# Maryamsana-1998/DiffCodec-Controlling-Latent-Diffusion-for-Perceptual-Video-Compression

Measured on AMD Instinct MI355X. Metric: decoded frames/sec @ 512x512, 20-step DDIM, GOP-12, higher is better.
Workload: dtype bf16; 1 GPU; 512x512 inter frames of a GOP-12 clip, 16 per step per GPU, 20-step DDIM, CFG 4.5 (model batch 32), control scale 1.7, SD-1.5 + DualFlowControlNet + VAE decode, random-init weights; hip_graphs=True, parallelism=unit-shard x1, backend=none, backend_world_size=1

## Files before the change

### diffcodec-controlling-latent-diffusion-for-perceptual-video-compression_amd/blocks.py

```python
import torch

from . import ops
from .ops import PackedConv


PROJ_IN_FUSE_MIN_ROWS = 1 << 62
PROJ_IN_GN_ON_LOAD = True
LN_FOLD = True


BUFFER_EPOCH = [0]


def _f32(sd, key, device):
    return sd[key].detach().float().contiguous().to(device)


class TimeEmbedding:

    def __init__(self, sd, device, ch0, resnet_prefixes):
        self.ch0 = ch0
        self.l1 = PackedConv(sd["time_embedding.linear_1.weight"], sd["time_embedding.linear_1.bias"], device)
        self.l2 = PackedConv(sd["time_embedding.linear_2.weight"], sd["time_embedding.linear_2.bias"], device)
        ws, bs, self.slices, off = [], [], {}, 0
# ... 19 lines not shown


class ResnetBlock:

    def __init__(self, sd, p, device, groups, eps):
        self.p, self.groups, self.eps = p, groups, eps
        self.n1 = (_f32(sd, p + "norm1.weight", device), _f32(sd, p + "norm1.bias", device))
        self.n2 = (_f32(sd, p + "norm2.weight", device), _f32(sd, p + "norm2.bias", device))
        self.conv1 = PackedConv(sd[p + "conv1.weight"], sd[p + "conv1.bias"], device)
        self.conv2 = PackedConv(sd[p + "conv2.weight"], sd[p + "conv2.bias"], device)
        self.shortcut = None
        if p + "conv_shortcut.weight" in sd:
            self.shortcut = PackedConv(sd[p + "conv_shortcut.weight"], sd[p + "conv_shortcut.bias"], device)

    def __call__(self, x, temb=None, x2=None):
        ab1 = ops.group_norm_ab(x, self.n1[0], self.n1[1], self.groups, self.eps, x2=x2)
        h = ops.conv_gn_silu(x, self.conv1, ab1, x2=x2, row_add=None if temb is None else temb.slice(self.p, x.shape[0]),
                             gn_part=True)
        ab2 = ops.group_norm_ab(h, self.n2[0], self.n2[1], self.groups, self.eps)
        if self.shortcut is not None:
            sc = ops.conv(x, self.shortcut, x2=x2)
        else:
            assert x2 is None
            sc = x
        return ops.conv_gn_silu(h, self.conv2, ab2, residual=sc, gn_part=True)


class TransformerBlock:

    def __init__(self, sd, p, device, heads, groups):
        self.heads, self.groups = heads, groups
        self.norm = (_f32(sd, p + "norm.weight", device), _f32(sd, p + "norm.bias", device))
        self.proj_in = PackedConv(sd[p + "proj_in.weight"], sd[p + "proj_in.bias"], device)
        self.proj_out = PackedConv(sd[p + "proj_out.weight"], sd[p + "proj_out.bias"], device)
        q = p + "transformer_blocks.0."
        self.ln = [(_f32(sd, q + f"norm{i}.weight", device), _f32(sd, q + f"norm{i}.bias", device)) for i in (1, 2, 3)]
        self.fold = LN_FOLD

        def ln(i):
            return (sd[q + f"norm{i}.weight"], sd[q + f"norm{i}.bias"], 1e-5) if self.fold else None
# ... 12 lines not shown
        new = ops.linear(ctx_bf16, self.kv2)
        if self.kv_ctx is not None and self.kv_ctx.shape == new.shape:
            self.kv_ctx.copy_(new)
        else:
            self.kv_ctx = new
            BUFFER_EPOCH[0] += 1

    def __call__(self, x, cfg_shared=False):
        n, h, w, c = x.shape
        fold = self.fold
        parts = ops.row_stats_parts(c) if fold else 0

        def stats_buf(rows):
            return torch.empty((rows, parts, 2), device=x.device, dtype=torch.float32) if fold else None

        ab = ops.group_norm_ab(x, self.norm[0], self.norm[1], self.groups, 1e-6)
        if PROJ_IN_GN_ON_LOAD and self.proj_in.bias is not None and ops.rowpanel_takes(n * h * w, h * w, c, self.proj_in.cout):
            st = stats_buf(n * h * w)
            t = ops.conv(x, self.proj_in, gn_ab=ab, gn_silu=False, stats_out=st).reshape(n, h * w, c)
        elif n * h * w > PROJ_IN_FUSE_MIN_ROWS:
            t = ops.conv(x, self.proj_in, gn_ab=ab, gn_silu=False).reshape(n, h * w, c)
            st = ops.row_stats(t) if fold else None
        else:
            st = stats_buf(n * h * w)
            t = ops.conv(ops.gn_apply(x, ab), self.proj_in, stats_out=st).reshape(n, h * w, c)
        qkv = ops.linear(t, self.qkv1, ln_partials=(st, 1e-5)) if fold else ops.linear(ops.layer_norm(t, *self.ln[0]), self.qkv1)
        a = ops.attention(qkv[..., :c], qkv[..., c:2 * c], qkv[..., 2 * c:], self.heads)
        st = stats_buf(n * h * w)
        t = ops.linear(a, self.out1, residual=t, stats_out=st)
        q = ops.linear(t, self.q2, ln_partials=(st, 1e-5)) if fold else ops.linear(ops.layer_norm(t, *self.ln[1]), self.q2)
        kv = self.kv_ctx
        if not cfg_shared:
            a = ops.attention(q, kv[..., :c], kv[..., c:], self.heads)
            st = stats_buf(n * h * w)
            t = ops.linear(a, self.out2, residual=t, stats_out=st)
        else:
            assert kv.shape[0] == 2 * n, "cfg_shared needs the [uncond | cond] context batch"
            a = torch.empty((2 * n, h * w, c), device=x.device, dtype=x.dtype)
            t2 = torch.empty_like(a)
            st = stats_buf(2 * n * h * w)
# ... 79 lines not shown
```

### diffcodec-controlling-latent-diffusion-for-perceptual-video-compression_amd/csrc/dc_conv_route.h

```cpp
#pragma once
#include "dc_common.h"
#include "../../include/diffcodec_hip.h"

struct dc_route {
    int kernel;
    int variant;
    int epi;
    int splitk;
    int ln_first;
    int tm, tn;
    int nst;
    int st;
    int gn;
    int ks3;
    int fast, ups, sh;
    int gn_chunks;
};

#define DC_ROUTE_PASS 1

static inline int dc_n_tile(const dc_conv_desc& d) { return (d.Cout % 160 == 0 && d.epilogue == 0) ? 160 : 128; }

int dc_gemm_dma_route(const dc_conv_desc& d, dc_route& r);
int dc_gemm_dma_launch(const dc_conv_desc& d, const dc_route& r, hipStream_t st);
int dc_gemm_rowpanel_route(const dc_conv_desc& d, dc_route& r);
int dc_gemm_rowpanel_launch(const dc_conv_desc& d, const dc_route& r, hipStream_t st);
int dc_gemm_p8_route(const dc_conv_desc& d, dc_route& r);
int dc_gemm_p8_launch(const dc_conv_desc& d, const dc_route& r, hipStream_t st);
int dc_gemm_wide_route(const dc_conv_desc& d, dc_route& r);
int dc_gemm_wide_launch(const dc_conv_desc& d, const dc_route& r, hipStream_t st);
int dc_conv3x3_tile_route(const dc_conv_desc& d, dc_route& r);
int dc_conv3x3_tile_launch(const dc_conv_desc& d, const dc_route& r, hipStream_t st);
```

### diffcodec-controlling-latent-diffusion-for-perceptual-video-compression_amd/csrc/igemm.hip

```cpp
#include "dc_conv_route.h"

namespace {

constexpr int BK = 64;

template <int WM, int WN, int TM, int TN, bool KS3, bool GN>
__global__ __launch_bounds__(256, 2) void igemm_kernel(const dc_conv_desc d)
{
    constexpr int BM = WM * TM * 16;
    constexpr int BN = WN * TN * 16;
    constexpr int PA = BM / 32;
    constexpr int PB = BN / 32;
    constexpr int A_BYTES = BM * 128;
    constexpr int B_BYTES = BN * 128;
    constexpr int BUF_BYTES = A_BYTES + B_BYTES;
    static_assert(WM * WN == 4, "4 waves");
    extern __shared__ __attribute__((aligned(16))) char smem[];

    const int tid = threadIdx.x;
    const int lane = tid & 63;
    const int wave = tid >> 6;
    const int wm = wave % WM;
    const int wn = wave / WM;
    const int q = tid & 7;
// ... 365 lines not shown
    if (d.row_add_stride == 0) d.row_add_stride = d.Cout;
    if (d.epilogue == 1 && (d.splitk > 1 || (d.Cout & 31) || d.residual || d.row_add || d.out_f32)) return DC_ERR_INVALID;
    const int asked = d.splitk, nkc = Cin >> 6;
    d.splitk = r.splitk = splitk_fixpoint(asked, nkc);
    int rc = dc_gemm_dma_route(d, r);
    if (rc == DC_ROUTE_PASS) rc = dc_conv3x3_tile_route(d, r);
    if (rc == DC_ROUTE_PASS) {
        d.splitk = r.splitk = splitk_fixpoint(asked, (d.ksize == 3 ? 9 : 1) * nkc);
        rc = igemm_route(d, r);
    }
    if (rc != DC_OK) return rc;
    if ((d.Cout & 15) && !(r.kernel == DC_ROUTE_CONV3X3_TILE && asked == 1)) return DC_ERR_INVALID;
    const bool gemm = r.kernel != DC_ROUTE_CONV3X3_TILE && r.kernel != DC_ROUTE_IGEMM;
    if ((d.ln_stats || d.stats_out) && !gemm) return DC_ERR_INVALID;
    if (d.gn_part_out && r.gn_chunks == 0) return DC_ERR_INVALID;
    return DC_OK;
}

}

extern "C" int dc_conv_gn_part_chunks(const dc_conv_desc* dp)
{
    if (!dp || dp->splitk > 1) return 0;
    dc_conv_desc q = *dp, d;
    if (!q.gn_part_out) q.gn_part_out = (float*)(uintptr_t)16;
    dc_route r;
    return conv_route(q, d, r) == DC_OK ? r.gn_chunks : 0;
}

extern "C" long long dc_conv_igemm_ws_bytes(const dc_conv_desc* d)
// ... 57 lines not shown
        rc = dc_ln_finalize(d.ln_stats, d.ln_scratch, (long long)d.N * d.Ho * d.Wo, d.ln_parts, d.C1 + d.C2, d.ln_eps, stream);
        if (rc != DC_OK) return rc;
        d.ln_stats = d.ln_scratch;
        d.ln_parts = 0;
    }
    switch (r.kernel) {
        case DC_ROUTE_GEMM_DMA: rc = dc_gemm_dma_launch(d, r, st); break;
        case DC_ROUTE_GEMM_WIDE: rc = dc_gemm_wide_launch(d, r, st); break;
        case DC_ROUTE_GEMM_P8: rc = dc_gemm_p8_launch(d, r, st); break;
        case DC_ROUTE_GEMM_ROWPANEL: rc = dc_gemm_rowpanel_launch(d, r, st); break;
        case DC_ROUTE_CONV3X3_TILE: rc = dc_conv3x3_tile_launch(d, r, st); break;
        default: rc = igemm_launch(d, r, st); break;
    }
    if (rc != DC_OK) return rc;
    if (d.splitk > 1) {
        const long long M = (long long)d.N * d.Ho * d.Wo;
        const long long total4 = M * d.Cout / 4;
        hipLaunchKernelGGL(splitk_finish_kernel, dim3(dc_cdiv(total4, 256)), dim3(256), 0, st, d, total4);
        return dc_launch_status();
    }
    return DC_OK;
}
```

### diffcodec-controlling-latent-diffusion-for-perceptual-video-compression_amd/csrc/norm.hip

```cpp
#include "dc_common.h"
#include "../../include/diffcodec_hip.h"

namespace {

__global__ __launch_bounds__(256) void gn_stats_kernel(const bf16_t* __restrict__ x, float* __restrict__ part,
                                                       long long HW, int C, int pix_per_block, int N)
{
    extern __shared__ float red[];
    const int nv = C >> 3;
    const int n = blockIdx.y;
    const long long p_begin = (long long)blockIdx.x * pix_per_block;
    const long long p_end = min(HW, p_begin + pix_per_block);
    const int tpp = min(nv, 256);
    const int ppb = 256 / tpp;
    const int vl = threadIdx.x % tpp, pl = threadIdx.x / tpp;
    if (pl < ppb) {
        for (int v = vl; v < nv; v += tpp) {
            float s[8], ss[8];
#pragma unroll
            for (int j = 0; j < 8; ++j) s[j] = ss[j] = 0.f;
            for (long long p0 = p_begin + pl; p0 < p_end; p0 += 4LL * ppb) {
                u32x4 raw[4];
#pragma unroll
                for (int u = 0; u < 4; ++u) {
// ... 175 lines not shown
                        continue;
                    }
                    float lo = __uint_as_float(raw[u][j] << 16) * g[j][0] + g[j][1];
                    float hi = __uint_as_float(raw[u][j] & 0xffff0000u) * g[j][2] + g[j][3];
                    lo = dc_silu(lo);
                    hi = dc_silu(hi);
                    bf16x2 pk = {(bf16_t)lo, (bf16_t)hi};
                    o[j] = *(uint32_t*)&pk;
                }
                *(u32x4*)(dst + p * C) = u32x4{o[0], o[1], o[2], o[3]};
            }
        }
    }
}

__global__ __launch_bounds__(256) void fdn_modulate_kernel(const bf16_t* __restrict__ x, const float* __restrict__ ab,
                                                           const bf16_t* __restrict__ gamma,
                                                           const bf16_t* __restrict__ beta, bf16_t* __restrict__ y,
                                                           int Bp, long long HW, int C, long long total_vec)
{
    const int nv = C >> 3;
    for (long long i = (long long)blockIdx.x * 256 + threadIdx.x; i < total_vec; i += (long long)gridDim.x * 256) {
        const long long pix = i / nv;
        const int c = (int)(i - pix * nv) * 8;
        const int n = (int)(pix / HW);
        const long long ppix = (long long)(n % Bp) * HW + (pix - (long long)n * HW);
        const bf16x8 xv = *(const bf16x8*)(x + pix * C + c);
        const bf16x8 gv = *(const bf16x8*)(gamma + ppix * C + c);
        const bf16x8 bv = *(const bf16x8*)(beta + ppix * C + c);
        const float* abp = ab + ((long long)n * C + c) * 2;
// ... 118 lines not shown
    if (!x1 || !ab || !y || N <= 0 || HW <= 0 || (C1 & 7) || (C2 & 7) || (C2 && !x2)) return DC_ERR_INVALID;
    const int nv = C >> 3, tpp = nv < 256 ? nv : 256, ppb = 256 / tpp;
    long long chunks = HW / (16LL * ppb);
    if (chunks < 1) chunks = 1;
    while (chunks * N < 1024 && chunks * 2 * 4 * ppb <= HW) chunks *= 2;
    const long long cap = 4096 / N > 0 ? 4096 / N : 1;
    if (chunks > cap) chunks = cap;
    if (chunks < 1) chunks = 1;
    const int pix_per_block = (int)((HW + chunks - 1) / chunks);
    const dim3 grid((unsigned)dc_cdiv(HW, pix_per_block), N);
    hipLaunchKernelGGL(gn_apply_kernel, grid, dim3(256), 0, (hipStream_t)stream, (const bf16_t*)x1, C1, (const bf16_t*)x2, C2, ab,
                       (bf16_t*)y, HW, pix_per_block, silu);
    return dc_launch_status();
}

extern "C" int dc_fdn_modulate_nhwc_bf16(const void* x, const float* ab, const void* gamma, const void* beta, void* y,
                                         int N, int Bp, long long HW, int C, void* stream)
{
    if (!x || !ab || !gamma || !beta || !y || N <= 0 || Bp <= 0 || HW <= 0 || (C & 7)) return DC_ERR_INVALID;
    const long long total_vec = (long long)N * HW * (C >> 3);
    const int grid = (int)min((long long)4096, (total_vec + 255) / 256);
    hipLaunchKernelGGL(fdn_modulate_kernel, dim3(grid), dim3(256), 0, (hipStream_t)stream, (const bf16_t*)x, ab,
                       (const bf16_t*)gamma, (const bf16_t*)beta, (bf16_t*)y, Bp, HW, C, total_vec);
    return dc_launch_status();
}

__global__ __launch_bounds__(256) void row_stats_kernel(const bf16_t* __restrict__ x, float* __restrict__ stats, long long M, int C)
{
    const int lane = threadIdx.x & 63;
    const long long row = (long long)blockIdx.x * 4 + (threadIdx.x >> 6);
// ... 57 lines not shown
```

### diffcodec-controlling-latent-diffusion-for-perceptual-video-compression_amd/lib.py

```python
import ctypes
import os
from ctypes import POINTER, c_double, c_float, c_int, c_longlong, c_void_p

HERE = os.path.dirname(os.path.abspath(__file__))
LIB_PATH = os.path.join(HERE, "libdiffcodec_hip.so")

vp, i32, i64, f32, f64 = c_void_p, c_int, c_longlong, c_float, c_double


class ConvDesc(ctypes.Structure):
    _fields_ = [
        ("x1", vp), ("x2", vp), ("w", vp), ("bias", vp), ("gn_ab", vp), ("row_add", vp), ("residual", vp),
        ("out", vp), ("splitk_ws", vp),
        ("N", i32), ("H", i32), ("W", i32), ("C1", i32), ("C2", i32), ("Cout", i32),
        ("ksize", i32), ("stride", i32), ("pad", i32), ("upsample", i32), ("Ho", i32), ("Wo", i32),
        ("gn_silu", i32), ("epilogue", i32), ("out_f32", i32), ("out_scale", f32), ("splitk", i32), ("gn_batch", i32),
        ("act", i32), ("row_add_stride", i64),
        ("ln_stats", vp), ("ln_colsum", vp), ("stats_out", vp), ("gn_part_out", vp),
        ("ln_parts", i32), ("ln_eps", f32), ("ln_scratch", vp),
    ]


SIGNATURES = {
    "dc_splat_soft_f32": [vp, vp, vp, vp, vp, vp, i32, i32, i32, i32, vp],
    "dc_splat_sum_f32": [vp, vp, vp, vp, i32, i32, i32, i32, vp],
    "dc_splat_ws_bytes": [i32, i32, i32],
    "dc_occlusion_mask_f32": [vp, vp, vp, vp, i32, i32, i32, vp],
    "dc_flow_resize_normalize_f32": [vp, i64, vp, i32, i32, i32, i32, i32, vp],
    "dc_flow_resize_divide_f32": [vp, i64, vp, i32, i32, i32, i32, i32, f32, f32, vp],
    "dc_fuse_warped_f32": [vp, vp, vp, vp, vp, vp, vp, i32, i32, i32, i32, vp],
    "dc_conv3x3_nchw_f32": [vp, i64, vp, vp, vp, i32, i32, i32, i32, i32, i32, i32, vp],
    "dc_conv3x3_f32_route": [i32, i32, i32, i32, i32, POINTER(i32)],
    "dc_nchw_f32_to_nhwc_bf16": [vp, vp, i32, i32, i32, i32, vp],
    "dc_nhwc_bf16_to_nchw_f32": [vp, vp, i32, i32, i32, i32, vp],
# ... 2 lines not shown
    "dc_conv_igemm_bf16": [POINTER(ConvDesc), vp],
    "dc_conv_route": [POINTER(ConvDesc), POINTER(i32)],
    "dc_conv_instance": [POINTER(ConvDesc), POINTER(i32)],
    "dc_conv_igemm_ws_bytes": [POINTER(ConvDesc)],
    "dc_gemm_row_stats_parts": [i32],
    "dc_conv_gn_part_chunks": [POINTER(ConvDesc)],
    "dc_row_stats_bf16": [vp, vp, i64, i32, vp],
    "dc_ln_finalize": [vp, vp, i64, i32, i32, f32, vp],
    "dc_conv_small_cin_bf16": [vp, vp, vp, vp, i32, i32, i32, i32, i32, i32, i32, i32, i32, i32, vp],
    "dc_conv_small_cout_bf16": [vp, vp, vp, vp, i32, i32, vp, i32, i32, i32, i32, i32, i32, i32, vp],
    "dc_gn_stats_nhwc_bf16": [vp, vp, i32, i64, i32, vp],
    "dc_gn_stats_chunks": [i64, i32],
    "dc_gn_finalize": [vp, i32, i32, vp, i32, i32, vp, vp, vp, i32, i32, i64, f32, vp],
    "dc_gn_direct_nhwc_bf16": [vp, i32, vp, i32, vp, vp, vp, i32, i64, i32, f32, vp],
    "dc_gn_apply_nhwc_bf16": [vp, i32, vp, i32, vp, vp, i32, i64, i32, vp],
    "dc_fdn_modulate_nhwc_bf16": [vp, vp, vp, vp, vp, i32, i32, i64, i32, vp],
    "dc_layernorm_bf16": [vp, vp, vp, vp, i64, i32, f32, vp],
    "dc_attention_bf16": [vp, vp, vp, vp, i32, i32, i32, i32, i32, i64, i64, i64, i64, f32, vp],
    "dc_attention_route": [i32, i32, i32, i32, i32, POINTER(i32)],
    "dc_attention_causal_small_bf16": [vp, vp, vp, vp, i32, i32, i32, i32, i64, i64, i64, i64, f32, vp],
    "dc_embed_tokens_bf16": [vp, vp, vp, vp, i32, i32, i32, i32, vp],
    "dc_softmax_rows_f32_to_bf16": [vp, vp, i64, i32, f32, vp],
    "dc_timestep_embedding_f32": [vp, vp, vp, i32, i32, vp],
    "dc_freeu_lowfreq_nhwc_bf16": [vp, vp, i32, i32, i32, i32, f32, vp],
    "dc_freeu_backbone_nhwc_bf16": [vp, vp, i64, i32, f32, vp],
    "dc_lincomb4_f32": [vp, vp, vp, vp, f32, f32, f32, f32, vp, i64, vp],
    "dc_transpose_bf16": [vp, vp, i32, i32, i32, vp],
    "dc_vae_sample_latents": [vp, vp, vp, f32, i32, i32, i32, i32, vp],
    "dc_silu_f32": [vp, vp, i64, vp],
    "dc_add_bf16": [vp, vp, vp, i64, vp],
# ... 105 lines not shown
```

### diffcodec-controlling-latent-diffusion-for-perceptual-video-compression_amd/ops.py

```python
import collections
import ctypes
import math

import torch

from . import lib
from .lib import ConvDesc

BF16 = torch.bfloat16
F32 = torch.float32


def _meta(family, shape, flops, nbytes):
    return (family, shape, float(flops), float(nbytes)) if lib.TIMER is not None else None



GN_DIRECT_MAX_PIXELS = 256
GN_EPILOGUE_STATS = True


def _stream():
    return torch.cuda.current_stream().cuda_stream


def _ptr(t):
    return 0 if t is None else t.data_ptr()


def _chk(t, dtype, name):
    if not t.is_cuda:
        raise ValueError(f"{name}: expected a device tensor (the HIP path has no CPU fallback)")
    if t.dtype != dtype:
# ... 133 lines not shown
def conv_instance(d):
    info = (ctypes.c_int * 9)()
    rc = lib.load().dc_conv_instance(d, info)
    if rc != 0:
        raise lib.HipLaunchError(f"dc_conv_instance returned {rc} (invalid argument)")
    kernel = ROUTE_NAMES[info[0]]
    return dict(zip(INSTANCE_ARGS[kernel], info[1:]), kernel=kernel)


def rowpanel_takes(rows, rows_per_sample, cin, cout):
    return cin == 320 and cout >= 320 and cout % 64 == 0 and rows >= 65536 and rows % 256 == 0 and rows_per_sample % 256 == 0


def conv(x1, pc, *, x2=None, gn_ab=None, gn_silu=False, row_add=None, residual=None, stride=1, pad=1,
         upsample=False, out_scale=1.0, out_f32=False, splitk=None, act=0, out=None, ln_stats=None, stats_out=None,
         gn_part=False, ln_partials=None):
    _chk(x1, BF16, "x1")
    n, h, w, c1 = x1.shape
    c2 = 0
    if x2 is not None:
        _chk(x2, BF16, "x2")
        assert x2.shape[:3] == x1.shape[:3]
        c2 = x2.shape[3]
    assert c1 + c2 == pc.cin, f"channel mismatch {c1}+{c2} vs {pc.cin}"
    k = pc.ksize
    if k == 1:
        ho, wo = h, w
    else:
        hin, win = (2 * h, 2 * w) if upsample else (h, w)
        ho = (hin + (2 if pad else 1) - 3) // stride + 1
        wo = (win + (2 if pad else 1) - 3) // stride + 1
# ... 63 lines not shown
        else:
            tile3 = k == 3 and stride == 1 and conv_route(d).kernel == "conv3x3_tile"
            splitk = _pick_splitk(m, pc.cout, kt, pc.cin // 64 if tile3 else None, rows_per_image=ho * wo)
        d.splitk = int(splitk)
    ws = torch.empty((splitk, m, pc.cout), device=x1.device, dtype=F32) if splitk > 1 else None
    d.splitk_ws = _ptr(ws)
    if ln_parts > 0 and conv_route(d).ln_first:
        ln_scratch = torch.empty((m, 2), device=x1.device, dtype=F32)
        d.ln_scratch = ln_scratch.data_ptr()
    part = None
    if gn_part and GN_EPILOGUE_STATS and not out_f32 and not pc.geglu and splitk == 1 and ln_stats is None:
        chunks = lib.load().dc_conv_gn_part_chunks(d)
        if chunks > 0:
            part = torch.empty((chunks, n, pc.cout, 2), device=x1.device, dtype=F32)
            d.gn_part_out = part.data_ptr()
    meta = None
    if lib.TIMER is not None:
        kk = pc.cin * k * k
        kernel = conv_route(d).kernel
        if kernel == "conv3x3_tile":
            fam = "conv3x3_tile_kernel (3x3 stride-1 halo-tile conv)"
        elif kernel == "igemm":
            fam = "igemm_kernel (strided / GN-on-load gather GEMM)"
        else:
            fam = "gemm_dma_kernel + gemm_wide_kernel + gemm_p8_kernel + gemm_rowpanel_kernel (1x1 conv / linear GEMM family)"
        nbytes = 2.0 * (n * h * w * pc.cin + pc.cout * kk + m * cout_eff * (2 if out_f32 else 1) + (m * pc.cout if residual is not None else 0))
        meta = _meta(fam, f"{k}x{k} s{stride} up{int(upsample)} M={m} N={pc.cout} K={kk} gn={int(gn_ab is not None)} geglu={int(pc.geglu)} "
                          f"ln={int(ln_stats is not None)} splitk={splitk}", 2.0 * m * pc.cout * kk, nbytes)
    lib.call("dc_conv_igemm_bf16", d, _stream(), meta=meta)
    if part is not None:
        out.gn_part = part
    return out


FUSE_GN_MAX_COUT = 160
FUSE_GN_SMALL_BATCH = 4


def conv_gn_silu(x, pc, ab, x2=None, **kw):
    if pc.kind == "igemm" and pc.ksize == 3 and pc.cout > FUSE_GN_MAX_COUT and x.shape[0] > FUSE_GN_SMALL_BATCH:
        return conv(gn_apply(x, ab, silu=True, x2=x2), pc, **kw)
    return conv(x, pc, x2=x2, gn_ab=ab, gn_silu=True, **kw)


def linear(x, pc, **kw):
    shp = x.shape
    y = conv(x.reshape(1, 1, -1, shp[-1]), pc, **kw)
    return y.reshape(*shp[:-1], y.shape[-1])


F32CONV_FORMS = {1: "mfma", 2: "blk", 3: "direct"}
F32ConvRoute = collections.namedtuple("F32ConvRoute", "form stride co_tile pixel_tile cols_t rows_t")


def conv3x3_f32_route(cin, h, w, cout, stride):
    info = (ctypes.c_int * 6)()
    rc = lib.load().dc_conv3x3_f32_route(int(cin), int(h), int(w), int(cout), int(stride), info)
# ... 46 lines not shown
        return gn_finalize(p1, gamma, beta, groups, hw, eps, p2)
    if hw > GN_DIRECT_MAX_PIXELS and (p1 is not None or p2 is not None):
        return gn_finalize(p1 if p1 is not None else gn_stats(x), gamma, beta, groups, hw, eps,
                           None if x2 is None else (p2 if p2 is not None else gn_stats(x2)))
    if hw <= GN_DIRECT_MAX_PIXELS and (c + c2) % groups == 0 and ((c + c2) // groups) % 2 == 0 and c % 2 == 0 and c2 % 2 == 0:
        _chk(x, BF16, "x")
        if x2 is not None:
            _chk(x2, BF16, "x2")
        ab = torch.empty((n, c + c2, 2), device=x.device, dtype=F32)
        lib.call("dc_gn_direct_nhwc_bf16", x.data_ptr(), c, _ptr(x2), c2, _ptr(gamma), _ptr(beta), ab.data_ptr(), n, hw,
                 groups, float(eps), _stream())
        return ab
    return gn_finalize(gn_stats(x), gamma, beta, groups, hw, eps, None if x2 is None else gn_stats(x2))


def gn_apply(x, ab, silu=False, x2=None):
    _chk(x, BF16, "x")
    n, c1 = x.shape[0], x.shape[-1]
    c2 = 0 if x2 is None else x2.shape[-1]
    hw = x.numel() // (n * c1)
    y = torch.empty(x.shape[:-1] + (c1 + c2,), device=x.device, dtype=BF16)
    lib.call("dc_gn_apply_nhwc_bf16", x.data_ptr(), c1, _ptr(x2), c2, ab.data_ptr(), y.data_ptr(), n, hw, int(silu), _stream(),
             meta=_meta("gn_apply_kernel (GroupNorm affine + SiLU)", f"N={n} HW={hw} C={c1}+{c2}", 4.0 * y.numel(), 4.0 * y.numel()))
    return y


def fdn_modulate(x, ab, gamma, beta):
    _chk(x, BF16, "x")
    _chk(gamma, BF16, "gamma")
    _chk(beta, BF16, "beta")
# ... 347 lines not shown
```

### include/diffcodec_hip.h

```cpp
#ifndef DIFFCODEC_HIP_H
#define DIFFCODEC_HIP_H
#include <stdint.h>
#ifdef __cplusplus
extern "C" {
#endif

long long dc_splat_ws_bytes(int N, int H, int W);
int dc_splat_soft_f32(const float* in, const float* flow, const float* metric, const float* mask,
                      float* out, void* ws, int N, int C, int H, int W, void* stream);
int dc_splat_sum_f32(const float* in, const float* flow, float* out, void* ws, int N, int C, int H, int W, void* stream);
int dc_occlusion_mask_f32(const float* flow_a, const float* flow_b, float* mask_out, void* ws,
                          int N, int H, int W, void* stream);
int dc_flow_resize_normalize_f32(const float* src, long long src_batch_stride, float* dst,
                                 int N, int H, int W, int h, int w, void* stream);
int dc_flow_resize_divide_f32(const float* src, long long src_batch_stride, float* dst, int N, int H, int W, int h, int w,
                              float div_x, float div_y, void* stream);
int dc_fuse_warped_f32(const float* warped_first, const float* warped_last, const float* conf_f,
                       const float* conf_b, const float* occ_f, const float* occ_b, float* fused,
                       int N, int C, int H, int W, void* stream);

int dc_conv3x3_nchw_f32(const float* x, long long x_batch_stride, const float* w, const float* bias, float* y,
                        int N, int Cin, int H, int W, int Cout, int stride, int silu, void* stream);
#define DC_F32CONV_ROUTE_INFO_INTS 6
#define DC_F32CONV_MFMA 1
// ... 26 lines not shown
    int gn_silu;
    int epilogue;
    int out_f32;
    float out_scale;
    int splitk;
    int gn_batch;
    int act;
    long long row_add_stride;
    const float* ln_stats;
    const float* ln_colsum;
    float* stats_out;
    float* gn_part_out;
    int ln_parts;
    float ln_eps;
    float* ln_scratch;
} dc_conv_desc;
int dc_conv_igemm_bf16(const dc_conv_desc* desc, void* stream);
#define DC_ROUTE_INFO_INTS 5
#define DC_ROUTE_GEMM_DMA 1
#define DC_ROUTE_GEMM_WIDE 2
#define DC_ROUTE_GEMM_P8 3
#define DC_ROUTE_GEMM_ROWPANEL 4
#define DC_ROUTE_CONV3X3_TILE 5
#define DC_ROUTE_IGEMM 6
int dc_conv_route(const dc_conv_desc* desc, int* info);
#define DC_CONV_INSTANCE_INTS 9
int dc_conv_instance(const dc_conv_desc* desc, int* info);
long long dc_conv_igemm_ws_bytes(const dc_conv_desc* desc);
int dc_gemm_row_stats_parts(int Cout);
int dc_conv_gn_part_chunks(const dc_conv_desc* desc);
// ... 2 lines not shown

int dc_conv_small_cin_bf16(const void* x, const void* w, const float* bias, void* out, int N, int H, int W,
                           int Cin, int Cout, int ksize, int stride, int pad, int Ho, int Wo, void* stream);
int dc_conv_small_cout_bf16(const void* x, const void* w, const float* bias, const float* gn_ab, int gn_silu,
                            int gn_batch, void* out, int out_f32, int N, int H, int W, int Cin, int Cout, int ksize,
                            void* stream);

int dc_gn_stats_chunks(long long HW, int C);
int dc_gn_stats_nhwc_bf16(const void* x, float* partials, int N, long long HW, int C, void* stream);
int dc_gn_finalize(const float* sums1, int C1, int chunks1, const float* sums2, int C2, int chunks2, const float* gamma,
                   const float* beta, float* ab, int N, int groups, long long HW, float eps, void* stream);
int dc_gn_direct_nhwc_bf16(const void* x1, int C1, const void* x2, int C2, const float* gamma, const float* beta,
                           float* ab, int N, long long HW, int groups, float eps, void* stream);
int dc_gn_apply_nhwc_bf16(const void* x1, int C1, const void* x2, int C2, const float* ab, void* y,
                          int N, long long HW, int silu, void* stream);
int dc_fdn_modulate_nhwc_bf16(const void* x, const float* ab, const void* gamma, const void* beta, void* y,
                              int N, int Bp, long long HW, int C, void* stream);
int dc_layernorm_bf16(const void* x, const float* gamma, const float* beta, void* y, long long M, int C, float eps,
                      void* stream);

int dc_attention_bf16(const void* q, const void* k, const void* v, void* out, int B, int heads, int Nq, int Nk, int D,
                      long long q_stride, long long k_stride, long long v_stride, long long o_stride, float scale,
                      void* stream);
#define DC_ATTN_ROUTE_INFO_INTS 5
int dc_attention_route(int B, int heads, int Nq, int Nk, int D, int* info);
int dc_attention_causal_small_bf16(const void* q, const void* k, const void* v, void* out, int B, int heads, int T, int D,
                                   long long q_stride, long long k_stride, long long v_stride, long long o_stride,
                                   float scale, void* stream);
int dc_embed_tokens_bf16(const long long* ids, const void* tok_emb, const void* pos_emb, void* out, int B, int T, int C,
                         int vocab, void* stream);
// ... 78 lines not shown
```

Before: 19.81 frames/s.

## Fuse GroupNorm stats, finalize and apply into one launch for small maps

Adds a gn_norm kernel that computes GroupNorm statistics and writes the normalized (optionally SiLU) output in one launch for small spatial maps, keeping the group's values in LDS. It also fuses the next ResNet norm into the split-K finish of conv1, so the split-K reduction produces both the conv output and the normalized input for conv2. The transformer proj_in path uses the one-launch norm too. This removes the separate stats, finalize and apply launches and their extra memory passes on low-resolution layers. In exchange it uses one block per (batch, group), which can limit parallelism, and adds LDS pressure.

```diff
diff --git a/diffcodec-controlling-latent-diffusion-for-perceptual-video-compression_amd/blocks.py b/diffcodec-controlling-latent-diffusion-for-perceptual-video-compression_amd/blocks.py
--- a/diffcodec-controlling-latent-diffusion-for-perceptual-video-compression_amd/blocks.py
+++ b/diffcodec-controlling-latent-diffusion-for-perceptual-video-compression_amd/blocks.py
@@ -57,16 +57,14 @@
             self.shortcut = PackedConv(sd[p + "conv_shortcut.weight"], sd[p + "conv_shortcut.bias"], device)
 
     def __call__(self, x, temb=None, x2=None):
-        ab1 = ops.group_norm_ab(x, self.n1[0], self.n1[1], self.groups, self.eps, x2=x2)
-        h = ops.conv_gn_silu(x, self.conv1, ab1, x2=x2, row_add=None if temb is None else temb.slice(self.p, x.shape[0]),
-                             gn_part=True)
-        ab2 = ops.group_norm_ab(h, self.n2[0], self.n2[1], self.groups, self.eps)
+        h = ops.gn_silu_conv(x, self.conv1, self.n1, self.groups, self.eps, x2=x2, gn_part=True, next_norm=(self.n2, self.conv2),
+                             row_add=None if temb is None else temb.slice(self.p, x.shape[0]))
         if self.shortcut is not None:
             sc = ops.conv(x, self.shortcut, x2=x2)
         else:
             assert x2 is None
             sc = x
-        return ops.conv_gn_silu(h, self.conv2, ab2, residual=sc, gn_part=True)
+        return ops.gn_silu_conv(h, self.conv2, self.n2, self.groups, self.eps, residual=sc, gn_part=True)
 
 
 class TransformerBlock:
@@ -109,8 +107,12 @@
         def stats_buf(rows):
             return torch.empty((rows, parts, 2), device=x.device, dtype=torch.float32) if fold else None
 
-        ab = ops.group_norm_ab(x, self.norm[0], self.norm[1], self.groups, 1e-6)
-        if PROJ_IN_GN_ON_LOAD and self.proj_in.bias is not None and ops.rowpanel_takes(n * h * w, h * w, c, self.proj_in.cout):
+        on_load = PROJ_IN_GN_ON_LOAD and self.proj_in.bias is not None and ops.rowpanel_takes(n * h * w, h * w, c, self.proj_in.cout)
+        xn = None
+        if not on_load and n * h * w <= PROJ_IN_FUSE_MIN_ROWS:
+            xn = ops.gn_norm(x, self.norm[0], self.norm[1], self.groups, 1e-6)
+        ab = ops.group_norm_ab(x, self.norm[0], self.norm[1], self.groups, 1e-6) if xn is None else None
+        if on_load:
             st = stats_buf(n * h * w)
             t = ops.conv(x, self.proj_in, gn_ab=ab, gn_silu=False, stats_out=st).reshape(n, h * w, c)
         elif n * h * w > PROJ_IN_FUSE_MIN_ROWS:
@@ -118,7 +120,7 @@
             st = ops.row_stats(t) if fold else None
         else:
             st = stats_buf(n * h * w)
-            t = ops.conv(ops.gn_apply(x, ab), self.proj_in, stats_out=st).reshape(n, h * w, c)
+            t = ops.conv(xn if xn is not None else ops.gn_apply(x, ab), self.proj_in, stats_out=st).reshape(n, h * w, c)
         qkv = ops.linear(t, self.qkv1, ln_partials=(st, 1e-5)) if fold else ops.linear(ops.layer_norm(t, *self.ln[0]), self.qkv1)
         a = ops.attention(qkv[..., :c], qkv[..., c:2 * c], qkv[..., 2 * c:], self.heads)
         st = stats_buf(n * h * w)
diff --git a/diffcodec-controlling-latent-diffusion-for-perceptual-video-compression_amd/csrc/dc_conv_route.h b/diffcodec-controlling-latent-diffusion-for-perceptual-video-compression_amd/csrc/dc_conv_route.h
--- a/diffcodec-controlling-latent-diffusion-for-perceptual-video-compression_amd/csrc/dc_conv_route.h
+++ b/diffcodec-controlling-latent-diffusion-for-perceptual-video-compression_amd/csrc/dc_conv_route.h
@@ -31,3 +31,5 @@
 int dc_gemm_wide_launch(const dc_conv_desc& d, const dc_route& r, hipStream_t st);
 int dc_conv3x3_tile_route(const dc_conv_desc& d, dc_route& r);
 int dc_conv3x3_tile_launch(const dc_conv_desc& d, const dc_route& r, hipStream_t st);
+int dc_gn_splitk_finish_takes(const dc_conv_desc& d);
+int dc_gn_splitk_finish_launch(const dc_conv_desc& d, hipStream_t st);
diff --git a/diffcodec-controlling-latent-diffusion-for-perceptual-video-compression_amd/csrc/igemm.hip b/diffcodec-controlling-latent-diffusion-for-perceptual-video-compression_amd/csrc/igemm.hip
--- a/diffcodec-controlling-latent-diffusion-for-perceptual-video-compression_amd/csrc/igemm.hip
+++ b/diffcodec-controlling-latent-diffusion-for-perceptual-video-compression_amd/csrc/igemm.hip
@@ -403,6 +403,7 @@
     const bool gemm = r.kernel != DC_ROUTE_CONV3X3_TILE && r.kernel != DC_ROUTE_IGEMM;
     if ((d.ln_stats || d.stats_out) && !gemm) return DC_ERR_INVALID;
     if (d.gn_part_out && r.gn_chunks == 0) return DC_ERR_INVALID;
+    if (d.gn_next_out && !dc_gn_splitk_finish_takes(d)) return DC_ERR_INVALID;
     return DC_OK;
 }
 
@@ -490,6 +491,7 @@
     }
     if (rc != DC_OK) return rc;
     if (d.splitk > 1) {
+        if (d.gn_next_out) return dc_gn_splitk_finish_launch(d, st);
         const long long M = (long long)d.N * d.Ho * d.Wo;
         const long long total4 = M * d.Cout / 4;
         hipLaunchKernelGGL(splitk_finish_kernel, dim3(dc_cdiv(total4, 256)), dim3(256), 0, st, d, total4);
diff --git a/diffcodec-controlling-latent-diffusion-for-perceptual-video-compression_amd/csrc/norm.hip b/diffcodec-controlling-latent-diffusion-for-perceptual-video-compression_amd/csrc/norm.hip
--- a/diffcodec-controlling-latent-diffusion-for-perceptual-video-compression_amd/csrc/norm.hip
+++ b/diffcodec-controlling-latent-diffusion-for-perceptual-video-compression_amd/csrc/norm.hip
@@ -1,4 +1,5 @@
 #include "dc_common.h"
+#include "dc_conv_route.h"
 #include "../../include/diffcodec_hip.h"
 
 namespace {
@@ -213,6 +214,220 @@
     }
 }
 
+enum { GN_READ = 0, GN_PARTS = 1, GN_SPLITK = 2 };
+
+struct gn_norm_args {
+    const bf16_t* x1;
+    const bf16_t* x2;
+    const float* s1;
+    const float* s2;
+    const float* gamma;
+    const float* beta;
+    bf16_t* y;
+    int C1, C2, chunks1, chunks2;
+    int N, HW, groups, tp, silu;
+    float inv_count, eps;
+};
+
+__device__ __forceinline__ void gn_accumulate_pair(uint32_t raw, float& s, float& ss)
+{
+#pragma clang fp contract(off)
+    const float lo = __uint_as_float(raw << 16), hi = __uint_as_float(raw & 0xffff0000u);
+    s += lo + hi;
+    ss += lo * lo + hi * hi;
+}
+
+__device__ __forceinline__ float2 gn_scale_shift(float s, float ss, float inv_count, float eps, float ga, float be)
+{
+#pragma clang fp contract(off)
+    const float mean = s * inv_count;
+    const float var = fmaxf(__builtin_fmaf(-mean, mean, ss * inv_count), 0.f);
+    const float rstd = rsqrtf(var + eps);
+    float2 o;
+    o.x = rstd * ga;
+    o.y = __builtin_fmaf(-(mean * rstd), ga, be);
+    return o;
+}
+
+__device__ __forceinline__ uint32_t gn_apply_pair(uint32_t raw, f32x4 g, int silu)
+{
+#pragma clang fp contract(off)
+    if (!silu) return dc_gn_affine_pair(raw, g);
+    const float lo = dc_silu(__builtin_fmaf(__uint_as_float(raw << 16), g[0], g[1]));
+    const float hi = dc_silu(__builtin_fmaf(__uint_as_float(raw & 0xffff0000u), g[2], g[3]));
+    const bf16x2 pk = {(bf16_t)lo, (bf16_t)hi};
+    return *(const uint32_t*)&pk;
+}
+
+__device__ __forceinline__ uint32_t gn_finish_pair(float2 v, float2 bv, float2 ra, bf16x2 rr, const dc_conv_desc& d)
+{
+#pragma clang fp contract(off)
+    if (d.bias) v.x += bv.x, v.y += bv.y;
+    if (d.row_add) v.x += ra.x, v.y += ra.y;
+    if (d.act) v.x = dc_act(v.x, d.act), v.y = dc_act(v.y, d.act);
+    if (d.residual) v.x = __builtin_fmaf(v.x, d.out_scale, (float)rr[0]), v.y = __builtin_fmaf(v.y, d.out_scale, (float)rr[1]);
+    else v.x *= d.out_scale, v.y *= d.out_scale;
+    const bf16x2 pk = {(bf16_t)v.x, (bf16_t)v.y};
+    return *(const uint32_t*)&pk;
+}
+
+template <int FORM>
+__global__ __launch_bounds__(256) void gn_norm_kernel(const gn_norm_args a, const dc_conv_desc d)
+{
+    constexpr int UB = 4;
+    extern __shared__ uint32_t vals[];
+    __shared__ float red[8];
+    __shared__ __attribute__((aligned(16))) float2 gab[512];
+    const int C1 = FORM == GN_SPLITK ? d.Cout : a.C1, C2 = FORM == GN_SPLITK ? 0 : a.C2;
+    const int C = C1 + C2, HW = a.HW, N = a.N;
+    const int n = blockIdx.x / a.groups, g = blockIdx.x - n * a.groups;
+    const int cpg = C / a.groups, g0 = g * cpg, hp = cpg >> 1;
+    const int a0 = min(g0, C1), a1 = min(g0 + cpg, C1);
+    const int b0 = max(g0, C1) - C1, b1 = max(g0 + cpg, C1) - C1;
+    const int w1 = a1 - a0, w2 = b1 - b0;
+    const int tid = threadIdx.x;
+    float s = 0.f, ss = 0.f;
+    if (FORM == GN_PARTS) {
+#pragma unroll 4
+        for (int i = tid; i < w1 * a.chunks1; i += 256) {
+            const int ch = i / w1, k = a0 + (i - ch * w1);
+            const float2 v = *(const float2*)(a.s1 + (((long long)ch * N + n) * C1 + k) * 2);
+            s += v.x;
+            ss += v.y;
+        }
+#pragma unroll 4
+        for (int i = tid; i < w2 * a.chunks2; i += 256) {
+            const int ch = i / w2, k = b0 + (i - ch * w2);
+            const float2 v = *(const float2*)(a.s2 + (((long long)ch * N + n) * C2 + k) * 2);
+            s += v.x;
+            ss += v.y;
+        }
+        s = dc_wave_sum(s);
+        ss = dc_wave_sum(ss);
+        if ((tid & 63) == 0) {
+            red[tid >> 6] = s;
+            red[4 + (tid >> 6)] = ss;
+        }
+        __syncthreads();
+        s = (red[0] + red[1]) + (red[2] + red[3]);
+        ss = (red[4] + red[5]) + (red[6] + red[7]);
+    } else {
+        const int tp = a.tp, j = tid % tp, pl = tid / tp, pstep = 256 / tp;
+        const int np = pl < HW ? (HW - pl + pstep - 1) / pstep : 0;
+        auto scan = [&](const bf16_t* __restrict__ x, int Cs, int c0, int c1, int q0) {
+            const int npairs = (c1 - c0) >> 1;
+            const int nq = j < npairs ? (npairs - j + tp - 1) / tp : 0;
+            const int total = np * nq;
+            for (int t0 = 0; t0 < total; t0 += UB) {
+                uint32_t raw[UB];
+                int li[UB], cc[UB];
+                long long off[UB];
+#pragma unroll
+                for (int u = 0; u < UB; ++u) {
+                    const int t = min(t0 + u, total - 1);
+                    const int pi = nq == 1 ? t : t / nq;
+                    const int p = pl + pi * pstep, q = j + (t - pi * nq) * tp;
+                    li[u] = p * hp + q0 + q;
+                    cc[u] = c0 + 2 * q;
+                    off[u] = ((long long)n * HW + p) * Cs + cc[u];
+                }
+                if (FORM == GN_READ) {
+#pragma unroll
+                    for (int u = 0; u < UB; ++u) raw[u] = *(const uint32_t*)(x + off[u]);
+                } else {
+                    const long long slab = (long long)N * HW * C;
+                    float2 v[UB], bv[UB], ra[UB];
+                    bf16x2 rr[UB];
+#pragma unroll
+                    for (int u = 0; u < UB; ++u) {
+                        const int c = cc[u];
+                        v[u] = *(const float2*)(d.splitk_ws + off[u]);
+                        bv[u] = d.bias ? *(const float2*)(d.bias + c) : float2{0.f, 0.f};
+                        ra[u] = d.row_add ? *(const float2*)(d.row_add + (long long)n * d.row_add_stride + c) : float2{0.f, 0.f};
+                        rr[u] = bf16x2{(bf16_t)0.f, (bf16_t)0.f};
+                        if (d.residual) rr[u] = *(const bf16x2*)((const bf16_t*)d.residual + off[u]);
+                    }
+                    int k = 1;
+                    for (; k + 2 <= d.splitk; k += 2) {
+                        float2 e0[UB], e1[UB];
+#pragma unroll
+                        for (int u = 0; u < UB; ++u) {
+                            e0[u] = *(const float2*)(d.splitk_ws + k * slab + off[u]);
+                            e1[u] = *(const float2*)(d.splitk_ws + (k + 1) * slab + off[u]);
+                        }
+#pragma unroll
+                        for (int u = 0; u < UB; ++u) {
+                            v[u].x += e0[u].x, v[u].y += e0[u].y;
+                            v[u].x += e1[u].x, v[u].y += e1[u].y;
+                        }
+                    }
+                    for (; k < d.splitk; ++k) {
+                        float2 e0[UB];
+#pragma unroll
+                        for (int u = 0; u < UB; ++u) e0[u] = *(const float2*)(d.splitk_ws + k * slab + off[u]);
+#pragma unroll
+                        for (int u = 0; u < UB; ++u) v[u].x += e0[u].x, v[u].y += e0[u].y;
+                    }
+#pragma unroll
+                    for (int u = 0; u < UB; ++u) {
+                        raw[u] = gn_finish_pair(v[u], bv[u], ra[u], rr[u], d);
+                        if (t0 + u < total) *(uint32_t*)((bf16_t*)d.out + off[u]) = raw[u];
+                    }
+                }
+#pragma unroll
+                for (int u = 0; u < UB; ++u)
+                    if (t0 + u < total) {
+                        gn_accumulate_pair(raw[u], s, ss);
+                        vals[li[u]] = raw[u];
+                    }
+            }
+        };
+        if (FORM == GN_SPLITK) {
+            scan(nullptr, C, g0, g0 + cpg, 0);
+        } else {
+            if (w1 > 0) scan(a.x1, C1, a0, a1, 0);
+            if (w2 > 0) scan(a.x2, C2, b0, b1, w1 >> 1);
+        }
+        s = dc_wave_sum(s);
+        ss = dc_wave_sum(ss);
+        if ((tid & 63) == 0) {
+            red[(tid >> 6) * 2] = s;
+            red[(tid >> 6) * 2 + 1] = ss;
+        }
+        __syncthreads();
+        s = red[0] + red[2] + red[4] + red[6];
+        ss = red[1] + red[3] + red[5] + red[7];
+    }
+    for (int k = tid; k < cpg; k += 256) {
+        const int c = g0 + k;
+        gab[k] = gn_scale_shift(s, ss, a.inv_count, a.eps, a.gamma ? a.gamma[c] : 1.f, a.beta ? a.beta[c] : 0.f);
+    }
+    __syncthreads();
+    const int items = HW * hp;
+    for (int i0 = tid; i0 < items; i0 += UB * 256) {
+        uint32_t raw[UB];
+        int qq[UB];
+        long long yo[UB];
+#pragma unroll
+        for (int u = 0; u < UB; ++u) {
+            const int i = min(i0 + u * 256, items - 1);
+            const int p = i / hp;
+            qq[u] = i - p * hp;
+            yo[u] = ((long long)n * HW + p) * C + g0 + 2 * qq[u];
+            if (FORM == GN_PARTS) {
+                const int c = 2 * qq[u];
+                raw[u] = c < w1 ? *(const uint32_t*)(a.x1 + ((long long)n * HW + p) * C1 + a0 + c)
+                                : *(const uint32_t*)(a.x2 + ((long long)n * HW + p) * C2 + b0 + (c - w1));
+            } else {
+                raw[u] = vals[i];
+            }
+        }
+#pragma unroll
+        for (int u = 0; u < UB; ++u)
+            if (i0 + u * 256 < items) *(uint32_t*)(a.y + yo[u]) = gn_apply_pair(raw[u], ((const f32x4*)gab)[qq[u]], a.silu);
+    }
+}
+
 __global__ __launch_bounds__(256) void fdn_modulate_kernel(const bf16_t* __restrict__ x, const float* __restrict__ ab,
                                                            const bf16_t* __restrict__ gamma,
                                                            const bf16_t* __restrict__ beta, bf16_t* __restrict__ y,
@@ -361,6 +576,59 @@
     return dc_launch_status();
 }
 
+extern "C" int dc_gn_norm_takes(long long HW, int C1, int C2, int groups)
+{
+    const long long C = (long long)C1 + C2;
+    if (HW <= 0 || groups <= 0 || C1 <= 0 || C2 < 0 || C % groups) return 0;
+    const long long cpg = C / groups;
+    if ((cpg & 1) || (C1 & 1) || (C2 & 1)) return 0;
+    return cpg <= 512 && HW * cpg * 2 <= 65536;
+}
+
+namespace {
+int gn_direct_tp(int cpg)
+{
+    const int npairs = cpg >> 1;
+    return npairs <= 8 ? 8 : (npairs <= 16 ? 16 : 32);
+}
+}
+
+extern "C" int dc_gn_norm_nhwc_bf16(const void* x1, int C1, const void* x2, int C2, const float* sums1, int chunks1,
+                                    const float* sums2, int chunks2, const float* gamma, const float* beta, void* y, int N,
+                                    long long HW, int groups, float eps, int silu, void* stream)
+{
+    if (!x1 || !y || N <= 0 || (C2 && !x2) || !dc_gn_norm_takes(HW, C1, C2, groups)) return DC_ERR_INVALID;
+    if (sums1 && (chunks1 <= 0 || (C2 && (!sums2 || chunks2 <= 0)))) return DC_ERR_INVALID;
+    if (!sums1 && sums2) return DC_ERR_INVALID;
+    const int cpg = (C1 + C2) / groups;
+    gn_norm_args a{};
+    a.x1 = (const bf16_t*)x1, a.x2 = (const bf16_t*)x2, a.s1 = sums1, a.s2 = sums2, a.gamma = gamma, a.beta = beta, a.y = (bf16_t*)y;
+    a.C1 = C1, a.C2 = C2, a.chunks1 = chunks1, a.chunks2 = C2 ? chunks2 : 0;
+    a.N = N, a.HW = (int)HW, a.groups = groups, a.tp = gn_direct_tp(cpg), a.silu = silu;
+    a.inv_count = 1.0f / ((float)HW * (float)cpg), a.eps = eps;
+    const dc_conv_desc none{};
+    if (sums1) hipLaunchKernelGGL(gn_norm_kernel<GN_PARTS>, dim3(N * groups), dim3(256), 0, (hipStream_t)stream, a, none);
+    else hipLaunchKernelGGL(gn_norm_kernel<GN_READ>, dim3(N * groups), dim3(256), (size_t)HW * cpg * 2, (hipStream_t)stream, a, none);
+    return dc_launch_status();
+}
+
+int dc_gn_splitk_finish_takes(const dc_conv_desc& d)
+{
+    return d.splitk > 1 && !d.out_f32 && d.epilogue == 0 &&
+           dc_gn_norm_takes((long long)d.Ho * d.Wo, d.Cout, 0, d.gn_next_groups);
+}
+
+int dc_gn_splitk_finish_launch(const dc_conv_desc& d, hipStream_t st)
+{
+    const int HW = d.Ho * d.Wo, cpg = d.Cout / d.gn_next_groups;
+    gn_norm_args a{};
+    a.gamma = d.gn_next_gamma, a.beta = d.gn_next_beta, a.y = (bf16_t*)d.gn_next_out;
+    a.N = d.N, a.HW = HW, a.groups = d.gn_next_groups, a.tp = gn_direct_tp(cpg), a.silu = d.gn_next_silu;
+    a.inv_count = 1.0f / ((float)HW * (float)cpg), a.eps = d.gn_next_eps;
+    hipLaunchKernelGGL(gn_norm_kernel<GN_SPLITK>, dim3(d.N * d.gn_next_groups), dim3(256), (size_t)HW * cpg * 2, st, a, d);
+    return dc_launch_status();
+}
+
 extern "C" int dc_fdn_modulate_nhwc_bf16(const void* x, const float* ab, const void* gamma, const void* beta, void* y,
                                          int N, int Bp, long long HW, int C, void* stream)
 {
diff --git a/diffcodec-controlling-latent-diffusion-for-perceptual-video-compression_amd/lib.py b/diffcodec-controlling-latent-diffusion-for-perceptual-video-compression_amd/lib.py
--- a/diffcodec-controlling-latent-diffusion-for-perceptual-video-compression_amd/lib.py
+++ b/diffcodec-controlling-latent-diffusion-for-perceptual-video-compression_amd/lib.py
@@ -18,6 +18,8 @@
         ("act", i32), ("row_add_stride", i64),
         ("ln_stats", vp), ("ln_colsum", vp), ("stats_out", vp), ("gn_part_out", vp),
         ("ln_parts", i32), ("ln_eps", f32), ("ln_scratch", vp),
+        ("gn_next_out", vp), ("gn_next_gamma", vp), ("gn_next_beta", vp),
+        ("gn_next_groups", i32), ("gn_next_silu", i32), ("gn_next_eps", f32),
     ]
 
 
@@ -50,6 +52,8 @@
     "dc_gn_finalize": [vp, i32, i32, vp, i32, i32, vp, vp, vp, i32, i32, i64, f32, vp],
     "dc_gn_direct_nhwc_bf16": [vp, i32, vp, i32, vp, vp, vp, i32, i64, i32, f32, vp],
     "dc_gn_apply_nhwc_bf16": [vp, i32, vp, i32, vp, vp, i32, i64, i32, vp],
+    "dc_gn_norm_takes": [i64, i32, i32, i32],
+    "dc_gn_norm_nhwc_bf16": [vp, i32, vp, i32, vp, i32, vp, i32, vp, vp, vp, i32, i64, i32, f32, i32, vp],
     "dc_fdn_modulate_nhwc_bf16": [vp, vp, vp, vp, vp, i32, i32, i64, i32, vp],
     "dc_layernorm_bf16": [vp, vp, vp, vp, i64, i32, f32, vp],
     "dc_attention_bf16": [vp, vp, vp, vp, i32, i32, i32, i32, i32, i64, i64, i64, i64, f32, vp],
diff --git a/diffcodec-controlling-latent-diffusion-for-perceptual-video-compression_amd/ops.py b/diffcodec-controlling-latent-diffusion-for-perceptual-video-compression_amd/ops.py
--- a/diffcodec-controlling-latent-diffusion-for-perceptual-video-compression_amd/ops.py
+++ b/diffcodec-controlling-latent-diffusion-for-perceptual-video-compression_amd/ops.py
@@ -17,6 +17,7 @@
 
 
 GN_DIRECT_MAX_PIXELS = 256
+GN_ONE_LAUNCH_MAX_PIXELS = 256
 GN_EPILOGUE_STATS = True
 
 
@@ -180,7 +181,7 @@
 
 def conv(x1, pc, *, x2=None, gn_ab=None, gn_silu=False, row_add=None, residual=None, stride=1, pad=1,
          upsample=False, out_scale=1.0, out_f32=False, splitk=None, act=0, out=None, ln_stats=None, stats_out=None,
-         gn_part=False, ln_partials=None):
+         gn_part=False, ln_partials=None, next_norm=None):
     _chk(x1, BF16, "x1")
     n, h, w, c1 = x1.shape
     c2 = 0
@@ -274,6 +275,13 @@
         if chunks > 0:
             part = torch.empty((chunks, n, pc.cout, 2), device=x1.device, dtype=F32)
             d.gn_part_out = part.data_ptr()
+    normed = None
+    if (next_norm is not None and splitk > 1 and not out_f32 and not pc.geglu and ho * wo <= min(GN_ONE_LAUNCH_MAX_PIXELS, GN_DIRECT_MAX_PIXELS)
+            and lib.load().dc_gn_norm_takes(ho * wo, pc.cout, 0, int(next_norm[2])) and conv_route(d).splitk > 1):
+        gamma, beta, groups, eps, silu = next_norm
+        normed = torch.empty((n, ho, wo, pc.cout), device=x1.device, dtype=BF16)
+        d.gn_next_out, d.gn_next_gamma, d.gn_next_beta = normed.data_ptr(), _ptr(gamma), _ptr(beta)
+        d.gn_next_groups, d.gn_next_silu, d.gn_next_eps = int(groups), int(bool(silu)), float(eps)
     meta = None
     if lib.TIMER is not None:
         kk = pc.cin * k * k
@@ -286,10 +294,12 @@
             fam = "gemm_dma_kernel + gemm_wide_kernel + gemm_p8_kernel + gemm_rowpanel_kernel (1x1 conv / linear GEMM family)"
         nbytes = 2.0 * (n * h * w * pc.cin + pc.cout * kk + m * cout_eff * (2 if out_f32 else 1) + (m * pc.cout if residual is not None else 0))
         meta = _meta(fam, f"{k}x{k} s{stride} up{int(upsample)} M={m} N={pc.cout} K={kk} gn={int(gn_ab is not None)} geglu={int(pc.geglu)} "
-                          f"ln={int(ln_stats is not None)} splitk={splitk}", 2.0 * m * pc.cout * kk, nbytes)
+                          f"ln={int(ln_stats is not None)} splitk={splitk}" + (" gn_next=1" if normed is not None else ""), 2.0 * m * pc.cout * kk, nbytes)
     lib.call("dc_conv_igemm_bf16", d, _stream(), meta=meta)
     if part is not None:
         out.gn_part = part
+    if normed is not None:
+        out.gn_next = (normed, _gn_key(*next_norm))
     return out
 
 
@@ -297,10 +307,26 @@
 FUSE_GN_SMALL_BATCH = 4
 
 
+def gn_apply_is_separate(pc, batch):
+    return pc.kind == "igemm" and pc.ksize == 3 and pc.cout > FUSE_GN_MAX_COUT and batch > FUSE_GN_SMALL_BATCH
+
+
 def conv_gn_silu(x, pc, ab, x2=None, **kw):
-    if pc.kind == "igemm" and pc.ksize == 3 and pc.cout > FUSE_GN_MAX_COUT and x.shape[0] > FUSE_GN_SMALL_BATCH:
+    if gn_apply_is_separate(pc, x.shape[0]):
         return conv(gn_apply(x, ab, silu=True, x2=x2), pc, **kw)
     return conv(x, pc, x2=x2, gn_ab=ab, gn_silu=True, **kw)
+
+
+def gn_silu_conv(x, pc, norm, groups, eps, x2=None, next_norm=None, **kw):
+    nn = None
+    if next_norm is not None and gn_apply_is_separate(next_norm[1], x.shape[0]):
+        nn = (next_norm[0][0], next_norm[0][1], groups, eps, True)
+    if gn_apply_is_separate(pc, x.shape[0]):
+        xn = gn_norm(x, norm[0], norm[1], groups, eps, silu=True, x2=x2)
+        if xn is not None:
+            return conv(xn, pc, next_norm=nn, **kw)
+    ab = group_norm_ab(x, norm[0], norm[1], groups, eps, x2=x2)
+    return conv_gn_silu(x, pc, ab, x2=x2, next_norm=nn, **kw)
 
 
 def linear(x, pc, **kw):
@@ -377,6 +403,39 @@
     return gn_finalize(gn_stats(x), gamma, beta, groups, hw, eps, None if x2 is None else gn_stats(x2))
 
 
+def _gn_key(gamma, beta, groups, eps, silu):
+    return (_ptr(gamma), _ptr(beta), int(groups), float(eps), bool(silu))
+
+
+def gn_norm(x, gamma, beta, groups, eps, silu=False, x2=None):
+    _chk(x, BF16, "x")
+    n, c = x.shape[0], x.shape[-1]
+    hw = x.numel() // (n * c)
+    c2 = 0
+    if x2 is not None:
+        _chk(x2, BF16, "x2")
+        c2 = x2.shape[-1]
+    nx = getattr(x, "gn_next", None)
+    if nx is not None and x2 is None and nx[1] == _gn_key(gamma, beta, groups, eps, silu):
+        return nx[0]
+    if hw > GN_ONE_LAUNCH_MAX_PIXELS or not lib.load().dc_gn_norm_takes(hw, c, c2, int(groups)):
+        return None
+    p1 = getattr(x, "gn_part", None)
+    p2 = None if x2 is None else getattr(x2, "gn_part", None)
+    if p1 is not None and (x2 is None or p2 is not None):
+        form = "parts"
+    elif hw <= GN_DIRECT_MAX_PIXELS:
+        form, p1, p2 = "read", None, None
+    else:
+        return None
+    y = torch.empty(x.shape[:-1] + (c + c2,), device=x.device, dtype=BF16)
+    lib.call("dc_gn_norm_nhwc_bf16", x.data_ptr(), c, _ptr(x2), c2, _ptr(p1), 0 if p1 is None else p1.shape[0], _ptr(p2),
+             0 if p2 is None else p2.shape[0], _ptr(gamma), _ptr(beta), y.data_ptr(), n, hw, int(groups), float(eps), int(bool(silu)),
+             _stream(), meta=_meta("gn_norm_kernel (one-launch GroupNorm + SiLU, small maps)", f"N={n} HW={hw} C={c}+{c2} {form}",
+                                   7.0 * y.numel(), 4.0 * y.numel()))
+    return y
+
+
 def gn_apply(x, ab, silu=False, x2=None):
     _chk(x, BF16, "x")
     n, c1 = x.shape[0], x.shape[-1]
diff --git a/include/diffcodec_hip.h b/include/diffcodec_hip.h
--- a/include/diffcodec_hip.h
+++ b/include/diffcodec_hip.h
@@ -64,6 +64,12 @@
     int ln_parts;
     float ln_eps;
     float* ln_scratch;
+    void* gn_next_out;
+    const float* gn_next_gamma;
+    const float* gn_next_beta;
+    int gn_next_groups;
+    int gn_next_silu;
+    float gn_next_eps;
 } dc_conv_desc;
 int dc_conv_igemm_bf16(const dc_conv_desc* desc, void* stream);
 #define DC_ROUTE_INFO_INTS 5
@@ -96,6 +102,10 @@
                            float* ab, int N, long long HW, int groups, float eps, void* stream);
 int dc_gn_apply_nhwc_bf16(const void* x1, int C1, const void* x2, int C2, const float* ab, void* y,
                           int N, long long HW, int silu, void* stream);
+int dc_gn_norm_takes(long long HW, int C1, int C2, int groups);
+int dc_gn_norm_nhwc_bf16(const void* x1, int C1, const void* x2, int C2, const float* sums1, int chunks1, const float* sums2,
+                         int chunks2, const float* gamma, const float* beta, void* y, int N, long long HW, int groups,
+                         float eps, int silu, void* stream);
 int dc_fdn_modulate_nhwc_bf16(const void* x, const float* ab, const void* gamma, const void* beta, void* y,
                               int N, int Bp, long long HW, int C, void* stream);
 int dc_layernorm_bf16(const void* x, const float* gamma, const float* beta, void* y, long long M, int C, float eps,
```

Result: no change. 19.76 frames/s (-0.2%).
